# PRBonn/kinematic-icp

Measured on NVIDIA H100. Metric: scans/sec (full ICP), higher is better.
Workload: dtype f64

## Files before the change

kinematic-icp_b200/csrc/kicp_register.cu:

```cuda
#include <cfloat>
#include <cmath>
#include <cstddef>
#include <cstdio>
#include <cstdlib>
#include <cstring>
#include <algorithm>

#include "kicp_register.cuh"
#include "kicp_solve.cuh"

using namespace kicp_dev;

#ifndef KR_WARPS
#define KR_WARPS 10
#endif
#define KR_THREADS (KR_WARPS * 32)
#ifndef KR_MINB
#define KR_MINB 2
#endif
#ifndef KR_LCAP
#define KR_LCAP 192
#endif
#ifndef KR_G
#define KR_G 3
#endif
#ifndef KR_MERGE_MAX
#define KR_MERGE_MAX 19
#endif
#ifndef KR_SLOWWIN
#define KR_SLOWWIN 8
#endif
#define KR_CLASSES 4
#ifndef KR_CLS_HEAVY
#define KR_CLS_HEAVY 8
#endif
#ifndef KR_CLS_MID
#define KR_CLS_MID 4
#endif
#define KR_DBLMAX_BITS 0x7FEFFFFFFFFFFFFFull
#ifdef KR_PROFILE
#define KR_PROF_DECL long long prof_t[24] = {0}; long long prof_last = clock64(); int prof_o = 0;
#define KR_PROF(i) { const long long t__ = clock64(); prof_t[prof_o + (i)] += t__ - prof_last; prof_last = t__; }
#define KR_PROF_COUNT(i) { prof_t[prof_o + (i)] += 1; }
#define KR_PROF_PASS(it) { prof_o = (it) ? 12 : 0; }
#define KR_PROF_FLUSH if (lane == 0) { for (int k__ = 0; k__ < 24; ++k__) atomicAdd(&st->prof[k__], (unsigned long long)prof_t[k__]); }
#define KR_WLOG_CAP 65536
__device__ unsigned long long g_wlog[KR_WLOG_CAP][4];
__device__ unsigned int g_wlog_n;
__device__ __forceinline__ unsigned smid() { unsigned r; asm volatile("mov.u32 %0, %%smid;" : "=r"(r)); return r; }
#define KR_WLOG(kind, t0, t1, a_, b_) if (lane == 0) { const unsigned i__ = atomicAdd(&g_wlog_n, 1u); if (i__ < KR_WLOG_CAP) { \
    g_wlog[i__][0] = (t0), g_wlog[i__][1] = (t1); \
    g_wlog[i__][2] = ((unsigned long long)(kind) << 56) | ((unsigned long long)it << 48) | ((unsigned long long)smid() << 32) | gwarp; \
    g_wlog[i__][3] = ((unsigned long long)(unsigned)(a_) << 32) | (unsigned)(b_); } }
#define KR_WLOG_DO(x) x
#else
#define KR_WLOG(kind, t0, t1, a_, b_)
#define KR_WLOG_DO(x)
#define KR_PROF_DECL
#define KR_PROF(i)
#define KR_PROF_COUNT(i)
#define KR_PROF_PASS(it)
#define KR_PROF_FLUSH
#endif

struct RegState {
    PoseState pose;
    unsigned int win_ctr;
    unsigned int arrive;
    unsigned int exit_ctr;
    unsigned int ticket;
    unsigned int a_arrive;
    union {
        unsigned int cls_n[KR_CLASSES][KICP_MAX_ITERATIONS];
        struct { unsigned int slow_n[KICP_MAX_ITERATIONS], heavy_n[KICP_MAX_ITERATIONS], mid_n[KICP_MAX_ITERATIONS], todo_n[KICP_MAX_ITERATIONS]; };
    };
    int abort;
    int *iters_out;
    double acc[8];
    unsigned long long stats[4];
    unsigned long long prof[24];
    double dbg[KICP_MAX_ITERATIONS][6];
    kicp_reg_result result;
};

#ifndef KR_EMU
__device__ __forceinline__ unsigned long long gtime_ns() {
    unsigned long long t;
    asm volatile("mov.u64 %0, %%globaltimer;" : "=l"(t));
    return t;
}
__device__ __forceinline__ uint32_t ld_acquire_sys_u32(const uint32_t *p) {
    uint32_t v;
    asm volatile("ld.acquire.sys.global.u32 %0, [%1];" : "=r"(v) : "l"(p) : "memory");
    return v;
}
__device__ __forceinline__ unsigned int ld_acquire_gpu_u32(const unsigned int *p) {
    unsigned int v;
    asm volatile("ld.acquire.gpu.global.u32 %0, [%1];" : "=r"(v) : "l"(p) : "memory");
    return v;
}
__device__ __forceinline__ void st_relaxed_sys_u64(unsigned long long *p, unsigned long long v) {
    asm volatile("st.relaxed.sys.global.u64 [%0], %1;" ::"l"(p), "l"(v) : "memory");
}
__device__ __forceinline__ unsigned long long ld_relaxed_sys_u64(const unsigned long long *p) {
    unsigned long long v;
    asm volatile("ld.relaxed.sys.global.u64 %0, [%1];" : "=l"(v) : "l"(p) : "memory");
    return v;
}
#endif
struct __align__(32) Point4 {
    double x, y, z, w;
};
#ifndef KR_EMU
__device__ __forceinline__ Point4 ld_point(const double *p) {
    Point4 r;
    asm volatile("ld.global.nc.v2.f64 {%0, %1}, [%2];" : "=d"(r.x), "=d"(r.y) : "l"(p));
    asm volatile("ld.global.nc.f64 %0, [%1];" : "=d"(r.z) : "l"(p + 2));
    r.w = 0.0;
    return r;
}
#endif

__global__ void k_reg_init(RegState *st, RegArgs a) {
    if (threadIdx.x != 0 || blockIdx.x != 0) return;
    pose_init(&st->pose, a);
    result_init(&st->result, &st->pose);
    st->ticket = 0, st->win_ctr = 0, st->arrive = 0, st->exit_ctr = 0, st->abort = 0, st->a_arrive = 0;
    for (int c = 0; c < KR_CLASSES; ++c)
        for (int k = 0; k < KICP_MAX_ITERATIONS; ++k) st->cls_n[c][k] = 0;
    st->iters_out = a.iters_out;
    if (a.iters_out) *a.iters_out = 0;
    for (int k = 0; k < 8; ++k) st->acc[k] = 0.0;
}

__global__ void k_solve(RegState *st) {
    if (threadIdx.x == 0 && blockIdx.x == 0 && !st->pose.done) {
        double s[8];
        for (int k = 0; k < 8; ++k) s[k] = st->acc[k];
        solve_and_update(&st->pose, s, &st->result, st->iters_out);
        for (int k = 0; k < 8; ++k) st->acc[k] = 0.0;
    }
}

#define KR_TCAP 640
struct __align__(8) LineDesc {
    unsigned gline;
    unsigned short owner;
    unsigned short nvalid;
};
struct __align__(16) WarpSm {
    double2 qxy[32];
    double qz[32];
    double lmin[KR_LCAP];
    LineDesc ldesc[KR_LCAP];
    int vx[32], vy[32], vz[32];
    double acc[7][32];
    double px[32], py[32];
    unsigned short task[KR_TCAP];
};

__device__ __noinline__ bool same_norm(double a, double b) { return sqrt(a) == sqrt(b); }
__device__ __forceinline__ bool closer(double d2, double best) {
    if (!(d2 < best)) return false;
    if (d2 >= best * (1.0 - 4e-16)) return !same_norm(d2, best);
    return true;
}

__device__ __forceinline__ double dist2(double cx, double cy, double cz, double qx, double qy, double qz) {
    const double dx = cx - qx, dy = cy - qy, dz = cz - qz;
    return add_rn(add_rn(__dmul_rn(dx, dx), __dmul_rn(dy, dy)), __dmul_rn(dz, dz));
}

__device__ __forceinline__ void query_rn(const double q[4], const double t[3], double px, double py, double pz, double &ox, double &oy,
                                         double &oz) {
    quat_rotate_rn(q[0], q[1], q[2], q[3], px, py, pz, ox, oy, oz);
    ox = add_rn(ox, t[0]), oy = add_rn(oy, t[1]), oz = add_rn(oz, t[2]);
}

__device__ __forceinline__ void load_scan_point(const ScanView &sv, int i, double &x, double &y, double &z) {
    const unsigned char *p = sv.base + (size_t)i * (size_t)sv.stride;
    if (sv.f32) {
        x = (double)__ldg(reinterpret_cast<const float *>(p + sv.ox));
        y = (double)__ldg(reinterpret_cast<const float *>(p + sv.oy));
        z = (double)__ldg(reinterpret_cast<const float *>(p + sv.oz));
    } else {
        x = __ldg(reinterpret_cast<const double *>(p + sv.ox));
        y = __ldg(reinterpret_cast<const double *>(p + sv.oy));
        z = __ldg(reinterpret_cast<const double *>(p + sv.oz));
    }
}

__device__ __forceinline__ void stats_flush(RegState *st, unsigned long long probes, unsigned long long cands, unsigned long long lines) {
#pragma unroll
    for (int d = 16; d > 0; d >>= 1) {
        probes += __shfl_xor_sync(0xFFFFFFFFu, probes, d);
        cands += __shfl_xor_sync(0xFFFFFFFFu, cands, d);
        lines += __shfl_xor_sync(0xFFFFFFFFu, lines, d);
    }
    if ((threadIdx.x & 31) == 0) atomicAdd(&st->stats[0], probes), atomicAdd(&st->stats[1], cands), atomicAdd(&st->stats[2], lines);
}

__device__ __forceinline__ unsigned stage_mask(int stage, bool valid, double bound, double qx, double qy, double qz, int vx, int vy,
                                               int vz, double vs, double &minpruned) {
    if (!valid) return 0u;
    if (stage == 0) return 1u;
    double t;
    t = (double)(vx + 1) * vs - qx; const double gxp = t * t;
    t = qx - (double)vx * vs;       const double gxm = t * t;
    t = (double)(vy + 1) * vs - qy; const double gyp = t * t;
    t = qy - (double)vy * vs;       const double gym = t * t;
    t = (double)(vz + 1) * vs - qz; const double gzp = t * t;
    t = qz - (double)vz * vs;       const double gzm = t * t;
    if (stage == 1) {
        unsigned mask = 0u;
        if (gxp <= bound) mask |= 1u << 1; else minpruned = fmin(minpruned, gxp);
        if (gxm <= bound) mask |= 1u << 2; else minpruned = fmin(minpruned, gxm);
        if (gyp <= bound) mask |= 1u << 3; else minpruned = fmin(minpruned, gyp);
        if (gym <= bound) mask |= 1u << 4; else minpruned = fmin(minpruned, gym);
        if (gzp <= bound) mask |= 1u << 5; else minpruned = fmin(minpruned, gzp);
        if (gzm <= bound) mask |= 1u << 6; else minpruned = fmin(minpruned, gzm);
        return mask;
    }
    unsigned mask = 0u;
#pragma unroll
    for (int kk = 7; kk < 27; ++kk) {
        const double lb2 = (shift_x(kk) > 0 ? gxp : (shift_x(kk) < 0 ? gxm : 0.0)) + (shift_y(kk) > 0 ? gyp : (shift_y(kk) < 0 ? gym : 0.0)) +
                           (shift_z(kk) > 0 ? gzp : (shift_z(kk) < 0 ? gzm : 0.0));
        if (lb2 <= bound) mask |= 1u << kk; else minpruned = fmin(minpruned, lb2);
    }
    return mask;
}

__device__ __forceinline__ unsigned seeded_near_mask(double sd, double tau, double qx, double qy, double qz, int vx, int vy, int vz, double vs,
                                                     double &minpruned) {
    const double seed2 = sd * sd * (1.0 + 1e-6);
    const double bound = fmin(tau * tau, seed2) * (1.0 + 1e-6) + 1e-10;
    return stage_mask(1, true, bound, qx, qy, qz, vx, vy, vz, vs, minpruned) | stage_mask(2, true, bound, qx, qy, qz, vx, vy, vz, vs, minpruned);
}

__device__ __forceinline__ unsigned *class_entry(const KernelArgs &a, int n, int c, unsigned pos) {
    unsigned *const base = (c == 0 || c == 3) ? a.todo : a.todo2;
    return base + ((c & 1) ? pos : (unsigned)n - 1u - pos);
}

__device__ __forceinline__ void accumulate(WarpSm &sm, int lane, const PoseState &ps, double nx, double ny, double nz, double qx, double qy,
                                           double qz, double px, double py) {
    const double rx = qx - nx, ry = qy - ny, rz = qz - nz;
    const double rr = rx * rx + ry * ry + rz * rz;
    if (sqrt(rr) < ps.tau) {
        const double c0x = ps.R[0], c0y = ps.R[3], c0z = ps.R[6];
        const double c1x = ps.R[1] * px - ps.R[0] * py, c1y = ps.R[4] * px - ps.R[3] * py, c1z = ps.R[7] * px - ps.R[6] * py;
        sm.acc[0][lane] += c0x * c0x + c0y * c0y + c0z * c0z;
        sm.acc[1][lane] += c0x * c1x + c0y * c1y + c0z * c1z;
        sm.acc[2][lane] += c1x * c1x + c1y * c1y + c1z * c1z;
        sm.acc[3][lane] += c0x * rx + c0y * ry + c0z * rz;
        sm.acc[4][lane] += c1x * rx + c1y * ry + c1z * rz;
        sm.acc[5][lane] += 1.0;
        sm.acc[6][lane] += rr;
    }
}

__device__ __forceinline__ int voxel_of(double x, double vs, double inv_vs, int pow2) {
    return pow2 ? (int)floor(x * inv_vs) : voxel_coord(x, vs);
}

template <bool PERSISTENT>
__global__ void __launch_bounds__(KR_THREADS, KR_MINB) k_register(const KernelArgs a) {
#ifndef KR_EMU
    extern __shared__ __align__(16) unsigned char s_dyn[];
#else
    __shared__ __align__(16) unsigned char s_dyn[KR_WARPS * sizeof(WarpSm)];
#endif
    __shared__ PoseState s_ps;
    __shared__ double s_part[KR_WARPS][8];
    __shared__ double s_sum[8];
    __shared__ int s_flag[2];
    __shared__ volatile int s_ncls[2];

    const int lane = threadIdx.x & 31, wid = threadIdx.x >> 5;
    const int quad = lane >> 2, sub = lane & 3;
    const unsigned FULL = 0xFFFFFFFFu;
    WarpSm &sm = reinterpret_cast<WarpSm *>(s_dyn)[wid];
    RegState *const st = a.st;
    const int n = a.scan.d_n ? min(__ldg(a.scan.d_n), a.scan.n) : a.scan.n;
    const int num_windows = (n + 31) >> 5;
    const unsigned total_warps = gridDim.x * KR_WARPS;
    const unsigned gwarp = blockIdx.x * KR_WARPS + (threadIdx.x >> 5);

    if (threadIdx.x == 0) {
        if (PERSISTENT) {
            pose_init(&s_ps, a.init);
            if (blockIdx.x == 0) {
                result_init(&st->result, &s_ps);
                if (a.init.iters_out) *a.init.iters_out = 0;
            }
        } else {
            s_ps = st->pose;
        }
    }
    __syncthreads();
    if (!PERSISTENT && s_ps.done) return;

    unsigned long long n_probe = 0, n_cand = 0, n_line = 0;
    unsigned tbase = 0;
    KR_PROF_DECL

    for (unsigned it = 0; !s_ps.done; ++it) {
#pragma unroll
        for (int k = 0; k < 7; ++k) sm.acc[k][lane] = 0.0;
        const unsigned long long t_iter0 = gtime_ns();
        KR_PROF_PASS(it)
        const double inv_vs = 1.0 / a.map.voxel_size;
        const int tpb = max(1, min(32, KR_LCAP / ((a.map.cap + 3) >> 2)));
        const bool cache = PERSISTENT && a.nn_g != nullptr;
        unsigned tk = 0;
        int nsearch = num_windows;
        unsigned long long t_a1 = t_iter0, t_a2 = t_iter0;

        if (cache && it > 0u) {
            for (int w = (int)gwarp; w < num_windows; w += (int)total_warps) {
                const int i = w * 32 + lane;
                const bool valid = i < n;
                double px = 0, py = 0, pz = 0;
                if (valid) load_scan_point(a.scan, i, px, py, pz);
                const unsigned g1 = valid ? __ldcg(&a.nn_g[i]) : 0xFFFFFFFFu;
                const unsigned g2 = valid ? __ldcg(&a.nn_g2[i]) : 0xFFFFFFFFu;
                const double l = valid ? (double)__ldcg(&a.nn_l[i]) : 0.0;
                const bool haveg = g1 != 0xFFFFFFFFu, have2 = g2 != 0xFFFFFFFFu;
                const Point4 c1 = ld_point(a.map.pts + (size_t)(haveg ? g1 : 0u) * KICP_PSTRIDE);
                const Point4 c2 = ld_point(a.map.pts + (size_t)(have2 ? g2 : 0u) * KICP_PSTRIDE);
                double qx, qy, qz, ox, oy, oz;
                query_rn(s_ps.q, s_ps.t, px, py, pz, qx, qy, qz);
                query_rn(s_ps.qp, s_ps.tp, px, py, pz, ox, oy, oz);
                const double vs = a.map.voxel_size;
                const int vx = voxel_of(qx, vs, inv_vs, a.pow2_voxel), vy = voxel_of(qy, vs, inv_vs, a.pow2_voxel),
                          vz = voxel_of(qz, vs, inv_vs, a.pow2_voxel);
                const int ovx = voxel_of(ox, vs, inv_vs, a.pow2_voxel), ovy = voxel_of(oy, vs, inv_vs, a.pow2_voxel),
                          ovz = voxel_of(oz, vs, inv_vs, a.pow2_voxel);
                const double mx = qx - ox, my = qy - oy, mz = qz - oz;
                const double delta = sqrt(mx * mx + my * my + mz * mz) * (1.0 + 1e-9) + 1e-12;
                const double d1 = sqrt(dist2(c1.x, c1.y, c1.z, qx, qy, qz));
                const double d2 = have2 ? sqrt(dist2(c2.x, c2.y, c2.z, qx, qy, qz)) : DBL_MAX;
                const bool second_wins = d2 < d1;
                const double dn = second_wins ? d2 : d1;
                const bool clear = !have2 || fabs(d1 - d2) > 1e-9 * (d1 + d2) + 1e-12;
                const Point4 c = second_wins ? c2 : c1;
                double slab = DBL_MAX;
                bool reach = true;
                if (vx != ovx || vy != ovy || vz != ovz) {
                    reach = abs(vx - ovx) <= 1 && abs(vy - ovy) <= 1 && abs(vz - ovz) <= 1;
                    if (vx > ovx) slab = fmin(slab, (double)(vx + 1) * vs - qx); else if (vx < ovx) slab = fmin(slab, qx - (double)vx * vs);
                    if (vy > ovy) slab = fmin(slab, (double)(vy + 1) * vs - qy); else if (vy < ovy) slab = fmin(slab, qy - (double)vy * vs);
                    if (vz > ovz) slab = fmin(slab, (double)(vz + 1) * vs - qz); else if (vz < ovz) slab = fmin(slab, qz - (double)vz * vs);
                    if (haveg)
                        reach = reach && abs(voxel_of(c1.x, vs, inv_vs, a.pow2_voxel) - vx) <= 1 && abs(voxel_of(c1.y, vs, inv_vs, a.pow2_voxel) - vy) <= 1 &&
                                abs(voxel_of(c1.z, vs, inv_vs, a.pow2_voxel) - vz) <= 1;
                    if (have2)
                        reach = reach && abs(voxel_of(c2.x, vs, inv_vs, a.pow2_voxel) - vx) <= 1 && abs(voxel_of(c2.y, vs, inv_vs, a.pow2_voxel) - vy) <= 1 &&
                                abs(voxel_of(c2.z, vs, inv_vs, a.pow2_voxel) - vz) <= 1;
                }
                const double room = fmin(l - delta, slab * (1.0 - 1e-9) - 1e-12);
                const bool cert = valid && reach && (haveg ? (clear && dn * (1.0 + 1e-9) + 1e-12 < room) : (room > s_ps.tau * (1.0 + 1e-9)));
                if (cert) {
                    a.nn_l[i] = __double2float_rz(room * (1.0 - 1e-7));
                    if (second_wins) a.nn_g[i] = g2, a.nn_g2[i] = g1;
                    if (haveg) accumulate(sm, lane, s_ps, c.x, c.y, c.z, qx, qy, qz, px, py);
                }
                const bool again = valid && !cert;
                int cls = -1;
                if (again) {
                    float seed = 3.0e38f;
                    if (haveg && abs(voxel_of(c.x, vs, inv_vs, a.pow2_voxel) - vx) <= 1 && abs(voxel_of(c.y, vs, inv_vs, a.pow2_voxel) - vy) <= 1 &&
                        abs(voxel_of(c.z, vs, inv_vs, a.pow2_voxel) - vz) <= 1)
                        seed = __double2float_ru(dn * (1.0 + 1e-7));
                    a.nn_l[i] = seed;
                    cls = 0;
                    if (seed < 1.0e38f) {
                        double mp = DBL_MAX;
                        const int near = __popc(seeded_near_mask((double)seed, s_ps.tau, qx, qy, qz, vx, vy, vz, vs, mp));
                        if (near <= KR_MERGE_MAX) cls = near + 1 >= KR_CLS_HEAVY ? 1 : near + 1 >= KR_CLS_MID ? 2 : 3;
                    }
                }
                unsigned need = 0u, cnt = 0u;
#pragma unroll
                for (int k = 0; k < KR_CLASSES; ++k) {
                    const unsigned m = __ballot_sync(FULL, cls == k);
                    if (cls == k) need = m;
                    if (lane == k) cnt = m;
                }
                unsigned pos = 0;
                if (cnt) pos = atomicAdd(&st->cls_n[lane][it], (unsigned)__popc(cnt));
                pos = __shfl_sync(FULL, pos, max(cls, 0)) + (unsigned)__popc(need & ((1u << lane) - 1u));
                if (cls >= 0) *class_entry(a, n, cls, pos) = (unsigned)i;
            }
            KR_WLOG(1, t_iter0, gtime_ns(), 0, 0)
            __syncthreads();
            if (threadIdx.x == 0) {
                t_a1 = gtime_ns();
                __threadfence();
                atomicAdd(&st->a_arrive, 1u);
                const unsigned target = it * gridDim.x;
                const unsigned long long deadline = gtime_ns() + a.timeout_ns;
                while (ld_acquire_gpu_u32(&st->a_arrive) < target) {
                    __nanosleep(20);
                    if (gtime_ns() > deadline) {
                        atomicExch(&st->abort, KICP_ERR_CUDA);
                        break;
                    }
                }
                t_a2 = gtime_ns();
                s_ncls[0] = (int)__ldcg(&st->cls_n[1][it]), s_ncls[1] = (int)__ldcg(&st->cls_n[2][it]);
            }
            __syncthreads();
        }
        const bool indirect = cache && it > 0u;
        const int nfast = indirect ? (int)(__ldcg(&st->cls_n[1][it]) + __ldcg(&st->cls_n[2][it]) + __ldcg(&st->cls_n[3][it])) : n;
        const int nslow = indirect ? (int)__ldcg(&st->cls_n[0][it]) : 0;
        const int P = (int)total_warps;
        const int nslowwin = (nslow + KR_SLOWWIN - 1) / KR_SLOWWIN;
        const int Pf = max(P - nslowwin, P / 2);
        int wsz = 32;
        if (PERSISTENT && nfast > 0) {
            if (nfast <= 32 * Pf) {
                wsz = max(1, (nfast + Pf - 1) / Pf);
            } else {
                const int rounds = (nfast + 32 * (P + nslowwin) - 1) / (32 * P);
                wsz = min(32, (nfast + rounds * Pf - 1) / (rounds * Pf));
            }
        }
        const int segpts = max(32, ((((n + 31) >> 5) + KICP_UPLOAD_CHUNKS - 1) / KICP_UPLOAD_CHUNKS) * 32);
        const int segwin = (segpts + wsz - 1) / wsz;
        int nfastwin;
        if (indirect) {
            nfastwin = (nfast + wsz - 1) / wsz;
        } else {
            const int nseg = min(KICP_UPLOAD_CHUNKS, (n + segpts - 1) / segpts), lastn = n - (nseg - 1) * segpts;
            nfastwin = n > 0 ? (nseg - 1) * segwin + (lastn + wsz - 1) / wsz : 0;
        }
        nsearch = nslowwin + nfastwin;

        int w = min((int)gwarp, nsearch);
        const unsigned dyn = (unsigned)max(nsearch - (int)total_warps, 0);
        KR_PROF(11)
        while (w < nsearch) {
            if (lane == 0) tk = atomicAdd(&st->win_ctr, 1u);
            KR_PROF_COUNT(8)
            KR_WLOG_DO(const unsigned long long wl_t0 = gtime_ns(); unsigned wl_tasks = 0; unsigned wl_lines = 0;)
            int slot, limit, seg_of_w = 0, wlanes = wsz, cls = 0;
            if (indirect) {
                if (w < nslowwin) {
                    slot = lane * nslowwin + w, limit = nslow, wlanes = KR_SLOWWIN;
                } else {
                    slot = lane * nfastwin + (w - nslowwin), limit = nfast, cls = 1;
                }
            } else {
                const int sgi = min(w / segwin, KICP_UPLOAD_CHUNKS - 1), lw = w - sgi * segwin;
                const int sbase = sgi * segpts, sn = min(segpts, n - sbase);
                const int sw = (sn + wsz - 1) / wsz;
                slot = sbase + lane * sw + lw, limit = lw < sw ? sbase + sn : 0;
                seg_of_w = sgi;
            }
            const bool valid = lane < wlanes && slot < limit;
            int pi = valid ? slot : 0;
            if (indirect) {
                int pos = slot;
                if (cls == 1 && pos >= s_ncls[0]) pos -= s_ncls[0], cls = 2;
                if (cls == 2 && pos >= s_ncls[1]) pos -= s_ncls[1], cls = 3;
                pi = valid ? (int)__ldcg(class_entry(a, n, cls, (unsigned)pos)) : 0;
            }
            if (PERSISTENT && a.up.flags != nullptr && it == 0u) {
                const uint32_t *f = a.up.flags + seg_of_w;
                const unsigned long long deadline = gtime_ns() + a.timeout_ns;
                bool pend = true;
                while (__any_sync(FULL, pend)) {
                    if (pend) {
                        if (ld_acquire_sys_u32(f) == a.up.seq) {
                            pend = false;
                        } else if (gtime_ns() > deadline) {
                            if (lane == 0) atomicExch(&st->abort, KICP_ERR_CUDA);
                            pend = false;
                        }
                    }
                }
            }
            double seed2 = DBL_MAX, seed_d = 3.0e38;
            {
                double px = 0, py = 0, pz = 0;
                if (valid) load_scan_point(a.scan, pi, px, py, pz);
                if (indirect && valid) {
                    const double sd = (double)__ldcg(&a.nn_l[pi]);
                    if (sd < 1.0e38) seed_d = sd, seed2 = sd * sd * (1.0 + 1e-6);
                }
                double qx, qy, qz;
                query_rn(s_ps.q, s_ps.t, px, py, pz, qx, qy, qz);
                sm.qxy[lane] = make_double2(qx, qy), sm.qz[lane] = qz;
                sm.vx[lane] = voxel_of(qx, a.map.voxel_size, inv_vs, a.pow2_voxel);
                sm.vy[lane] = voxel_of(qy, a.map.voxel_size, inv_vs, a.pow2_voxel);
                sm.vz[lane] = voxel_of(qz, a.map.voxel_size, inv_vs, a.pow2_voxel);
                sm.px[lane] = px, sm.py[lane] = py;
            }
            double best = DBL_MAX, second = DBL_MAX, third = DBL_MAX, minpruned = DBL_MAX;
            unsigned bline = 0xFFFFFFFFu, bvalid = 0u;
            unsigned sline = 0xFFFFFFFFu, svalid = 0u;
            __syncwarp();
            KR_PROF(0)

            unsigned donem = 0u;
            bool merged = false;
            for (int stage = 0; stage < 3; ++stage) {
                if (stage == 1 && !__any_sync(FULL, valid && !merged)) break;
                int total, tfirst, tcount;
                {
                    const double2 qq = sm.qxy[lane];
                    const double tau2 = s_ps.tau * s_ps.tau;
                    const double bsq = fmin(fmin(tau2, best), seed2);
                    const double bound = bsq * (1.0 + 1e-6) + 1e-10;
                    unsigned mask = stage_mask(stage, valid, bound, qq.x, qq.y, sm.qz[lane], sm.vx[lane], sm.vy[lane], sm.vz[lane],
                                               a.map.voxel_size, minpruned);
                    if (stage == 0 && valid && seed_d < 1.0e38) {
                        double mp = minpruned;
                        const unsigned near = seeded_near_mask(seed_d, s_ps.tau, qq.x, qq.y, sm.qz[lane], sm.vx[lane], sm.vy[lane], sm.vz[lane],
                                                               a.map.voxel_size, mp);
                        if (__popc(near) <= KR_MERGE_MAX) mask |= near, minpruned = mp, merged = true;
                    }
                    mask &= ~donem;
                    donem |= mask;
                    const int no = __popc(mask);
                    int tin = no;
#pragma unroll
                    for (int d = 1; d < 32; d <<= 1) {
                        const int y = __shfl_up_sync(FULL, tin, d);
                        if (lane >= d) tin += y;
                    }
                    total = __shfl_sync(FULL, tin, 31);
                    int pos = tin - no;
                    tfirst = pos, tcount = no;
                    const int maxno = __reduce_max_sync(FULL, no);
                    for (int i = 0; i < maxno; ++i) {
                        if (mask) {
                            const int k = __ffs(mask) - 1;
                            mask &= mask - 1;
                            sm.task[pos++] = (unsigned short)((lane << 5) | k);
                        }
                    }
                    __syncwarp();
                }
                KR_PROF(1)
                KR_WLOG_DO(wl_tasks += (unsigned)total;)
                int fill = 0, lbase = 0;
                int olb = 0, ole = 0;
                bool ohas = false;
                for (int base = 0;; base += tpb) {
                    const bool more = base < total;
                    const bool act = more && lane < tpb && base + lane < total;
                    const unsigned okpack = act ? (unsigned)sm.task[base + lane] : 0u;
                    uint32_t meta = KICP_SLOT_EMPTY;
                    if (more) {
                        KR_PROF_COUNT(9)
                        const int o = (int)(okpack >> 5), k = (int)(okpack & 31u);
                        const int kx = sm.vx[o] + shift_x(k), ky = sm.vy[o] + shift_y(k), kz = sm.vz[o] + shift_z(k);
                        uint32_t h = voxel_hash(kx, ky, kz) & a.map.mask;
                        const int4 s0 = __ldg(&a.map.slots[h]);
                        const int4 s1 = __ldg(&a.map.slots[(h + 1) & a.map.mask]);
                        bool pend = false;
                        if (act && (uint32_t)s0.w != KICP_SLOT_EMPTY) {
                            if (s0.x == kx && s0.y == ky && s0.z == kz) {
                                meta = (uint32_t)s0.w;
                            } else if ((uint32_t)s1.w != KICP_SLOT_EMPTY) {
                                if (s1.x == kx && s1.y == ky && s1.z == kz) {
                                    meta = (uint32_t)s1.w;
                                } else {
                                    pend = true, h = (h + 2) & a.map.mask;
                                }
                            }
                        }
                        while (__any_sync(FULL, pend)) {
                            if (pend) {
                                const int4 sl = __ldg(&a.map.slots[h]);
                                if ((uint32_t)sl.w == KICP_SLOT_EMPTY) {
                                    pend = false;
                                } else if (sl.x == kx && sl.y == ky && sl.z == kz) {
                                    meta = (uint32_t)sl.w, pend = false;
                                } else {
                                    h = (h + 1) & a.map.mask;
                                }
                            }
                        }
                    }
                    KR_PROF(2)
                    const int cnt = meta == KICP_SLOT_EMPTY ? 0 : (int)(meta & 0xFFu);
                    const int nl = (cnt + 3) >> 2;
                    int incl = nl;
#pragma unroll
                    for (int d = 1; d < 32; d <<= 1) {
                        const int y = __shfl_up_sync(FULL, incl, d);
                        if (lane >= d) incl += y;
                    }
                    const int ltot = __shfl_sync(FULL, incl, 31);
                    if (a.collect_stats) n_probe += act ? 1 : 0, n_cand += cnt, n_line += nl;

                    if ((!more || fill + ltot > KR_LCAP) && fill > 0) {
                        KR_PROF(3)
                        for (int r0 = 0; r0 < fill; r0 += 8 * KR_G) {
                            unsigned own[KR_G], gix[KR_G];
                            unsigned hasm = 0;
#pragma unroll
                            for (int g = 0; g < KR_G; ++g) {
                                const int line = r0 + g * 8 + quad;
                                LineDesc ld;
                                ld.gline = 0u, ld.owner = 0, ld.nvalid = 0;
                                if (line < fill) ld = sm.ldesc[line];
                                const bool has = sub < (int)ld.nvalid;
                                own[g] = ld.owner;
                                gix[g] = ld.gline + (has ? (unsigned)sub : 0u);
                                hasm |= has ? (1u << g) : 0u;
                            }
                            Point4 c[KR_G];
#pragma unroll
                            for (int g = 0; g < KR_G; ++g) c[g] = ld_point(a.map.pts + (size_t)gix[g] * KICP_PSTRIDE);
                            KR_PROF_COUNT(10)
                            KR_PROF(4)
#pragma unroll
                            for (int g = 0; g < KR_G; ++g) {
                                const double2 qq = sm.qxy[own[g]];
                                double d2 = (hasm >> g) & 1u ? dist2(c[g].x, c[g].y, c[g].z, qq.x, qq.y, sm.qz[own[g]]) : DBL_MAX;
                                d2 = fmin(d2, __shfl_xor_sync(FULL, d2, 1));
                                d2 = fmin(d2, __shfl_xor_sync(FULL, d2, 2));
                                if (sub == 0 && r0 + g * 8 + quad < fill) sm.lmin[r0 + g * 8 + quad] = d2;
                            }
                        }
                        __syncwarp();
                        {
                            const int lb = ohas ? max(olb - lbase, 0) : 0, le = ohas ? min(ole - lbase, fill) : 0;
                            const int maxlen = __reduce_max_sync(FULL, max(le - lb, 0));
                            for (int u = 0; u < maxlen; ++u) {
                                if (lb + u < le) {
                                    const double dl = sm.lmin[lb + u];
                                    if (closer(dl, best)) {
                                        const LineDesc ld = sm.ldesc[lb + u];
                                        third = second;
                                        second = best, sline = bline, svalid = bvalid;
                                        best = dl, bline = ld.gline, bvalid = ld.nvalid;
                                    } else if (dl < second) {
                                        const LineDesc ld = sm.ldesc[lb + u];
                                        third = second;
                                        second = dl, sline = ld.gline, svalid = ld.nvalid;
                                    } else {
                                        third = fmin(third, dl);
                                    }
                                }
                            }
                        }
                        __syncwarp();
                        KR_WLOG_DO(wl_lines += (unsigned)fill;)
                        lbase += fill, fill = 0;
                        KR_PROF(5)
                    }
                    if (!more) break;
                    {
                        const int gl = lbase + fill + (incl - nl);
                        const int t0 = max(tfirst - base, 0), t1 = min(tfirst + tcount - base, tpb);
                        const int b0 = __shfl_sync(FULL, gl, t0 & 31), e1 = __shfl_sync(FULL, gl + nl, (t1 - 1) & 31);
                        if (t1 > t0) {
                            if (!ohas) olb = b0, ohas = true;
                            ole = e1;
                        }
                        const int maxnl = __reduce_max_sync(FULL, nl);
                        for (int li = 0; li < maxnl; ++li) {
                            if (li < nl) {
                                LineDesc ld;
                                ld.gline = (meta >> 8) * (unsigned)a.map.cap + (unsigned)(li * 4);
                                ld.owner = (unsigned short)(okpack >> 5);
                                ld.nvalid = (unsigned short)min(cnt - li * 4, 4);
                                sm.ldesc[gl - lbase + li] = ld;
                            }
                        }
                        fill += ltot;
                    }
                    __syncwarp();
                    KR_PROF(3)
                }
                __syncwarp();
            }
            KR_PROF(1)
            {
                const bool have = valid && bline != 0xFFFFFFFFu;
                const unsigned g0 = have ? bline : 0u;
                Point4 cc[4];
#pragma unroll
                for (int j = 0; j < 4; ++j) cc[j] = ld_point(a.map.pts + (size_t)(g0 + (j < (int)bvalid ? j : 0)) * KICP_PSTRIDE);
                const double2 q0 = sm.qxy[lane];
                const double q0z = sm.qz[lane];
                double dj[4];
#pragma unroll
                for (int j = 0; j < 4; ++j) dj[j] = dist2(cc[j].x, cc[j].y, cc[j].z, q0.x, q0.y, q0z);
                int jw = 0;
#pragma unroll
                for (int j = 1; j < 4; ++j)
                    if (j < (int)bvalid && closer(dj[j], dj[jw])) jw = j;
                Point4 c = cc[0];
#pragma unroll
                for (int j = 1; j < 4; ++j)
                    if (jw == j) c = cc[j];
                if (have) accumulate(sm, lane, s_ps, c.x, c.y, c.z, q0.x, q0.y, q0z, sm.px[lane], sm.py[lane]);
                if (cache && valid) {
                    const bool have2 = have && sline != 0xFFFFFFFFu;
                    Point4 ce[4];
#pragma unroll
                    for (int j = 0; j < 4; ++j) ce[j] = ld_point(a.map.pts + (size_t)((have2 ? sline : 0u) + (j < (int)svalid ? j : 0)) * KICP_PSTRIDE);
                    double ru = DBL_MAX, ru2 = DBL_MAX;
                    unsigned g2 = 0xFFFFFFFFu;
#pragma unroll
                    for (int j = 0; j < 4; ++j) {
                        if (have && j < (int)bvalid && j != jw) {
                            if (dj[j] < ru) ru2 = ru, ru = dj[j], g2 = g0 + (unsigned)j;
                            else ru2 = fmin(ru2, dj[j]);
                        }
                    }
#pragma unroll
                    for (int j = 0; j < 4; ++j) {
                        const double de = dist2(ce[j].x, ce[j].y, ce[j].z, q0.x, q0.y, q0z);
                        if (have2 && j < (int)svalid) {
                            if (de < ru) ru2 = ru, ru = de, g2 = sline + (unsigned)j;
                            else ru2 = fmin(ru2, de);
                        }
                    }
                    const double lo2 = fmin(fmin(ru2, third), minpruned);
                    a.nn_g[pi] = have ? g0 + (unsigned)jw : 0xFFFFFFFFu;
                    a.nn_g2[pi] = g2;
                    a.nn_l[pi] = lo2 >= 1.0e60 ? 1.0e30f : __double2float_rz(sqrt(lo2) * (1.0 - 1e-7));
                }
            }
            __syncwarp();
            KR_PROF(6)
            KR_WLOG_DO(const unsigned wl_pts = (unsigned)__popc(__ballot_sync(FULL, valid));)
            KR_WLOG(0, wl_t0, gtime_ns(), (wl_tasks << 8) | wl_pts, wl_lines)
            w = (int)(total_warps + min(__shfl_sync(FULL, tk, 0) - tbase, dyn));
            KR_PROF(7)
        }
        tbase += (unsigned)nsearch;
        KR_PROF(11)

        const unsigned long long t_win = gtime_ns();
        double v[7];
#pragma unroll
        for (int k = 0; k < 7; ++k) v[k] = sm.acc[k][lane];
#pragma unroll
        for (int k = 0; k < 7; ++k) {
#pragma unroll
            for (int d = 16; d > 0; d >>= 1) v[k] += __shfl_xor_sync(FULL, v[k], d);
        }
        if (lane == 0) {
#pragma unroll
            for (int k = 0; k < 7; ++k) s_part[wid][k] = v[k];
            s_part[wid][7] = 0.0;
        }
        __syncthreads();
        double *const part = a.partials + (size_t)(PERSISTENT ? (it & 1u) : 0u) * gridDim.x * 8;
        if (threadIdx.x < 8) {
            double s = 0.0;
            for (int k = 0; k < KR_WARPS; ++k) s += s_part[k][threadIdx.x];
            __stcg(&part[(size_t)blockIdx.x * 8 + threadIdx.x], s);
            __threadfence();
        }
        __syncthreads();

        if (!PERSISTENT) {
            if (threadIdx.x == 0) {
                const unsigned ticket = atomicAdd(&st->ticket, 1u);
                s_flag[0] = (ticket == gridDim.x - 1);
            }
            __syncthreads();
            if (s_flag[0]) {
                __threadfence();
                if (threadIdx.x < 8) {
                    double s = 0.0;
                    for (unsigned bb = 0; bb < gridDim.x; ++bb) s += __ldcg(&part[(size_t)bb * 8 + threadIdx.x]);
                    st->acc[threadIdx.x] = s;
                }
                if (threadIdx.x == 0) st->ticket = 0, st->win_ctr = 0;
            }
            if (a.collect_stats) stats_flush(st, n_probe, n_cand, n_line);
            return;
        }

        const bool multi = a.px.nranks > 1;
        unsigned long long t_arr = 0, t_red = 0;
        if (threadIdx.x == 0) {
            atomicAdd(&st->arrive, 1u);
            if (!multi || blockIdx.x == 0) {
                const unsigned target = (it + 1u) * gridDim.x;
                const unsigned long long deadline = t_win + a.timeout_ns;
                while (ld_acquire_gpu_u32(&st->arrive) < target) {
                    __nanosleep(40);
                    if (gtime_ns() > deadline) {
                        atomicExch(&st->abort, KICP_ERR_CUDA);
                        break;
                    }
                }
            }
            t_arr = gtime_ns();
        }
        __syncthreads();
        if (!multi || blockIdx.x == 0) {
            const int col = threadIdx.x & 7, row0 = threadIdx.x >> 3;
            double s = 0.0;
            const unsigned nrow = (gridDim.x + KR_THREADS / 8 - 1) / (KR_THREADS / 8);
            for (unsigned kr = 0; kr < nrow; ++kr) {
                const unsigned bb = kr * (KR_THREADS / 8) + (unsigned)row0;
                if (bb < gridDim.x) s += __ldcg(&part[(size_t)bb * 8 + col]);
            }
            s += __shfl_xor_sync(FULL, s, 8);
            s += __shfl_xor_sync(FULL, s, 16);
            if (lane < 8) s_part[wid][lane] = s;
            __syncthreads();
            if (threadIdx.x < 8) {
                double tsum = 0.0;
                for (int k = 0; k < KR_WARPS; ++k) tsum += s_part[k][threadIdx.x];
                s_sum[threadIdx.x] = tsum;
            }
            __syncthreads();
        }
        if (multi) {
            const uint32_t tag = a.px.tag_base + it;
            if (wid == 0) {
                if (blockIdx.x == 0) {
                    const double val = s_sum[(lane & 15) >> 1];
                    const unsigned long long bits = (unsigned long long)__double_as_longlong(val);
                    const uint32_t half = (lane & 1) ? (uint32_t)(bits >> 32) : (uint32_t)bits;
                    const unsigned long long word = ((unsigned long long)tag << 32) | half;
#pragma unroll 1
                    for (int r = 0; r < a.px.nranks; ++r) {
                        st_relaxed_sys_u64(&a.px.peer[r]->ll[a.px.parity][it][a.px.rank][lane & 15], word);
                        __syncwarp();
                    }
                }
                __syncwarp();
                double tot = 0.0;
                bool timed_out = false;
                const unsigned long long deadline = gtime_ns() + a.timeout_ns;
                for (int r = 0; r < a.px.nranks; ++r) {
                    unsigned long long wv = 0;
                    const unsigned long long *src = &a.px.peer[a.px.rank]->ll[a.px.parity][it][r][lane & 15];
                    bool pend = true;
                    while (__any_sync(FULL, pend)) {
                        if (pend) {
                            wv = ld_relaxed_sys_u64(src);
                            if ((uint32_t)(wv >> 32) == tag) {
                                pend = false;
                            } else if (gtime_ns() > deadline) {
                                timed_out = true, pend = false;
                            }
                        }
                    }
                    const uint32_t lo = __shfl_sync(FULL, (uint32_t)wv, (lane & 7) * 2);
                    const uint32_t hi = __shfl_sync(FULL, (uint32_t)wv, (lane & 7) * 2 + 1);
                    tot += __longlong_as_double((long long)(((unsigned long long)hi << 32) | lo));
                }
                timed_out = __any_sync(FULL, timed_out);
                if (lane < 8) s_sum[lane] = tot;
                if (lane == 0) s_flag[1] = timed_out ? 1 : 0;
            }
            __syncthreads();
        }
        if (threadIdx.x == 0) {
            t_red = gtime_ns();
            int ab = (int)ld_acquire_gpu_u32((const unsigned int *)&st->abort);
            if (!ab && multi && s_flag[1]) ab = KICP_ERR_NCCL;
            if (ab) {
                s_ps.status = ab, s_ps.done = 1;
                if (blockIdx.x == 0) st->result.status = ab;
            } else {
                double s[8];
                for (int k = 0; k < 8; ++k) s[k] = s_sum[k];
                solve_and_update(&s_ps, s, blockIdx.x == 0 ? &st->result : nullptr, blockIdx.x == 0 ? a.init.iters_out : nullptr);
            }
            if (blockIdx.x == 0 && it < KICP_MAX_ITERATIONS) {
                st->dbg[it][0] = (double)(t_a1 - t_iter0), st->dbg[it][1] = (double)(t_a2 - t_a1), st->dbg[it][2] = (double)(t_win - t_a2);
                st->dbg[it][3] = (double)(t_arr - t_win), st->dbg[it][4] = (double)(t_red - t_arr), st->dbg[it][5] = (double)(gtime_ns() - t_red);
            }
        }
        __syncthreads();
    }

    if (PERSISTENT) {
        if (a.collect_stats) stats_flush(st, n_probe, n_cand, n_line);
        KR_PROF_FLUSH
        __syncthreads();
        if (blockIdx.x == 0 && a.result_host != nullptr) {
            const double *src = reinterpret_cast<const double *>(&st->result);
            double *dst = reinterpret_cast<double *>(a.result_host);
            for (unsigned i = threadIdx.x; i < sizeof(kicp_reg_result) / sizeof(double); i += KR_THREADS) dst[i] = __ldcg(src + i);
            __threadfence_system();
        }
        if (threadIdx.x == 0) {
            __threadfence();
            const unsigned left = atomicAdd(&st->exit_ctr, 1u);
            if (left == gridDim.x - 1) {
                st->win_ctr = 0, st->arrive = 0, st->abort = 0, st->a_arrive = 0;
                for (int c = 0; c < KR_CLASSES; ++c)
                    for (int k = 0; k < KICP_MAX_ITERATIONS; ++k) st->cls_n[c][k] = 0;
                __threadfence();
                st->exit_ctr = 0;
            }
        }
    }
}


#ifndef KR_EMU
__global__ void k_l2_read(const uint4 *__restrict__ p, size_t n, int reps, unsigned *sink) {
    unsigned acc = 0;
    for (int r = 0; r < reps; ++r)
        for (size_t i = (size_t)blockIdx.x * blockDim.x + threadIdx.x; i < n; i += (size_t)gridDim.x * blockDim.x) {
            const uint4 v = __ldcg(p + i);
            acc += v.x ^ v.y ^ v.z ^ v.w;
        }
    if (acc == 0x12345678u) *sink = acc;
}
size_t kr_state_bytes() { return sizeof(RegState); }
size_t kr_offset_result() { return offsetof(RegState, result); }
size_t kr_offset_acc() { return offsetof(RegState, acc); }
size_t kr_offset_dbg() { return offsetof(RegState, dbg); }
size_t kr_offset_stats() { return offsetof(RegState, stats); }
size_t kr_stats_bytes() { return sizeof(((RegState *)0)->stats) + sizeof(((RegState *)0)->prof); }
size_t kr_smem_bytes() { return (size_t)KR_WARPS * sizeof(WarpSm); }

cudaError_t kr_prepare(int *persistent_ctas_per_sm, int *multilaunch_ctas_per_sm) {
    cudaError_t e = cudaFuncSetAttribute(k_register<true>, cudaFuncAttributeMaxDynamicSharedMemorySize, (int)kr_smem_bytes());
    if (e == cudaSuccess) e = cudaFuncSetAttribute(k_register<false>, cudaFuncAttributeMaxDynamicSharedMemorySize, (int)kr_smem_bytes());
    if (e == cudaSuccess) e = cudaOccupancyMaxActiveBlocksPerMultiprocessor(persistent_ctas_per_sm, k_register<true>, KR_THREADS, kr_smem_bytes());
    if (e == cudaSuccess) e = cudaOccupancyMaxActiveBlocksPerMultiprocessor(multilaunch_ctas_per_sm, k_register<false>, KR_THREADS, kr_smem_bytes());
    return e;
}
cudaError_t kr_launch_init(RegState *st, const RegArgs &a, cudaStream_t stream) {
    k_reg_init<<<1, 32, 0, stream>>>(st, a);
    return cudaGetLastError();
}
cudaError_t kr_launch_solve(RegState *st, cudaStream_t stream) {
    k_solve<<<1, 32, 0, stream>>>(st);
    return cudaGetLastError();
}
cudaError_t kr_window_log(unsigned long long *out, size_t cap_entries, size_t *n) {
    *n = 0;
#ifdef KR_PROFILE
    unsigned cnt = 0;
    cudaError_t e = cudaMemcpyFromSymbol(&cnt, g_wlog_n, sizeof(cnt));
    if (e != cudaSuccess) return e;
    *n = std::min<size_t>(std::min<size_t>(cnt, KR_WLOG_CAP), cap_entries);
    return cudaMemcpyFromSymbol(out, g_wlog, *n * 4 * sizeof(unsigned long long));
#else
    (void)out, (void)cap_entries;
    return cudaSuccess;
#endif
}
cudaError_t kr_launch_register(bool persistent, int grid, KernelArgs &ka, cudaStream_t stream) {
#ifdef KR_PROFILE
    {
        void *p = nullptr;
        cudaGetSymbolAddress(&p, g_wlog_n);
        cudaMemsetAsync(p, 0, sizeof(unsigned), stream);
    }
#endif
    if (persistent) {
        void *args[] = {&ka};
        return cudaLaunchCooperativeKernel((const void *)k_register<true>, dim3(grid), dim3(KR_THREADS), args, kr_smem_bytes(), stream);
    }
    k_register<false><<<grid, KR_THREADS, kr_smem_bytes(), stream>>>(ka);
    return cudaGetLastError();
}
cudaError_t kr_launch_l2_read(const void *buf, size_t bytes, int reps, unsigned *sink, int grid, cudaStream_t stream) {
    k_l2_read<<<grid, 256, 0, stream>>>((const uint4 *)buf, bytes / 16, reps, sink);
    return cudaGetLastError();
}
#endif
```

Measured before the change: 3027.

## Batch cached-certify windows per warp with prefetch and one atomic per sweep

The cached-correspondence certify pass now handles up to eight grid-strided windows per warp in a sweep. It prefetches the next window's scan point and cached indices while certifying the current one. Class counts are accumulated across the sweep, so one atomicAdd per class reserves slots for all windows, followed by a second pass that writes the class entries. The abort flag is also read right after the arrival spin rather than with a separate acquire load later, which could weaken memory ordering for the single-rank path.

```diff
diff --git a/kinematic-icp_b200/csrc/kicp_register.cu b/kinematic-icp_b200/csrc/kicp_register.cu
--- a/kinematic-icp_b200/csrc/kicp_register.cu
+++ b/kinematic-icp_b200/csrc/kicp_register.cu
@@ -31,6 +31,7 @@
 #define KR_SLOWWIN 8
 #endif
 #define KR_CLASSES 4
+#define KR_SWEEP 8
 #ifndef KR_CLS_HEAVY
 #define KR_CLS_HEAVY 8
 #endif
@@ -264,6 +265,64 @@
     return pow2 ? (int)floor(x * inv_vs) : voxel_coord(x, vs);
 }
 
+__device__ __forceinline__ int certify(const KernelArgs &a, const PoseState &ps, WarpSm &sm, int lane, int i, bool valid, double px, double py,
+                                       double pz, unsigned g1, unsigned g2, double l, const Point4 &c1, const Point4 &c2, double inv_vs) {
+    const bool haveg = g1 != 0xFFFFFFFFu, have2 = g2 != 0xFFFFFFFFu;
+    double qx, qy, qz, ox, oy, oz;
+    query_rn(ps.q, ps.t, px, py, pz, qx, qy, qz);
+    query_rn(ps.qp, ps.tp, px, py, pz, ox, oy, oz);
+    const double vs = a.map.voxel_size;
+    const int vx = voxel_of(qx, vs, inv_vs, a.pow2_voxel), vy = voxel_of(qy, vs, inv_vs, a.pow2_voxel),
+              vz = voxel_of(qz, vs, inv_vs, a.pow2_voxel);
+    const int ovx = voxel_of(ox, vs, inv_vs, a.pow2_voxel), ovy = voxel_of(oy, vs, inv_vs, a.pow2_voxel),
+              ovz = voxel_of(oz, vs, inv_vs, a.pow2_voxel);
+    const double mx = qx - ox, my = qy - oy, mz = qz - oz;
+    const double delta = sqrt(mx * mx + my * my + mz * mz) * (1.0 + 1e-9) + 1e-12;
+    const double d1 = sqrt(dist2(c1.x, c1.y, c1.z, qx, qy, qz));
+    const double d2 = have2 ? sqrt(dist2(c2.x, c2.y, c2.z, qx, qy, qz)) : DBL_MAX;
+    const bool second_wins = d2 < d1;
+    const double dn = second_wins ? d2 : d1;
+    const bool clear = !have2 || fabs(d1 - d2) > 1e-9 * (d1 + d2) + 1e-12;
+    const Point4 c = second_wins ? c2 : c1;
+    double slab = DBL_MAX;
+    bool reach = true;
+    if (vx != ovx || vy != ovy || vz != ovz) {
+        reach = abs(vx - ovx) <= 1 && abs(vy - ovy) <= 1 && abs(vz - ovz) <= 1;
+        if (vx > ovx) slab = fmin(slab, (double)(vx + 1) * vs - qx); else if (vx < ovx) slab = fmin(slab, qx - (double)vx * vs);
+        if (vy > ovy) slab = fmin(slab, (double)(vy + 1) * vs - qy); else if (vy < ovy) slab = fmin(slab, qy - (double)vy * vs);
+        if (vz > ovz) slab = fmin(slab, (double)(vz + 1) * vs - qz); else if (vz < ovz) slab = fmin(slab, qz - (double)vz * vs);
+        if (haveg)
+            reach = reach && abs(voxel_of(c1.x, vs, inv_vs, a.pow2_voxel) - vx) <= 1 && abs(voxel_of(c1.y, vs, inv_vs, a.pow2_voxel) - vy) <= 1 &&
+                    abs(voxel_of(c1.z, vs, inv_vs, a.pow2_voxel) - vz) <= 1;
+        if (have2)
+            reach = reach && abs(voxel_of(c2.x, vs, inv_vs, a.pow2_voxel) - vx) <= 1 && abs(voxel_of(c2.y, vs, inv_vs, a.pow2_voxel) - vy) <= 1 &&
+                    abs(voxel_of(c2.z, vs, inv_vs, a.pow2_voxel) - vz) <= 1;
+    }
+    const double room = fmin(l - delta, slab * (1.0 - 1e-9) - 1e-12);
+    const bool cert = valid && reach && (haveg ? (clear && dn * (1.0 + 1e-9) + 1e-12 < room) : (room > ps.tau * (1.0 + 1e-9)));
+    if (cert) {
+        a.nn_l[i] = __double2float_rz(room * (1.0 - 1e-7));
+        if (second_wins) a.nn_g[i] = g2, a.nn_g2[i] = g1;
+        if (haveg) accumulate(sm, lane, ps, c.x, c.y, c.z, qx, qy, qz, px, py);
+    }
+    const bool again = valid && !cert;
+    int cls = -1;
+    if (again) {
+        float seed = 3.0e38f;
+        if (haveg && abs(voxel_of(c.x, vs, inv_vs, a.pow2_voxel) - vx) <= 1 && abs(voxel_of(c.y, vs, inv_vs, a.pow2_voxel) - vy) <= 1 &&
+            abs(voxel_of(c.z, vs, inv_vs, a.pow2_voxel) - vz) <= 1)
+            seed = __double2float_ru(dn * (1.0 + 1e-7));
+        a.nn_l[i] = seed;
+        cls = 0;
+        if (seed < 1.0e38f) {
+            double mp = DBL_MAX;
+            const int near = __popc(seeded_near_mask((double)seed, ps.tau, qx, qy, qz, vx, vy, vz, vs, mp));
+            if (near <= KR_MERGE_MAX) cls = near + 1 >= KR_CLS_HEAVY ? 1 : near + 1 >= KR_CLS_MID ? 2 : 3;
+        }
+    }
+    return cls;
+}
+
 template <bool PERSISTENT>
 __global__ void __launch_bounds__(KR_THREADS, KR_MINB) k_register(const KernelArgs a) {
 #ifndef KR_EMU
@@ -318,80 +377,49 @@
         unsigned long long t_a1 = t_iter0, t_a2 = t_iter0;
 
         if (cache && it > 0u) {
-            for (int w = (int)gwarp; w < num_windows; w += (int)total_warps) {
-                const int i = w * 32 + lane;
-                const bool valid = i < n;
+            for (int w0 = (int)gwarp; w0 < num_windows; w0 += KR_SWEEP * (int)total_warps) {
+                const int kn = min(KR_SWEEP, (num_windows - 1 - w0) / (int)total_warps + 1);
+                int i = w0 * 32 + lane;
                 double px = 0, py = 0, pz = 0;
-                if (valid) load_scan_point(a.scan, i, px, py, pz);
-                const unsigned g1 = valid ? __ldcg(&a.nn_g[i]) : 0xFFFFFFFFu;
-                const unsigned g2 = valid ? __ldcg(&a.nn_g2[i]) : 0xFFFFFFFFu;
-                const double l = valid ? (double)__ldcg(&a.nn_l[i]) : 0.0;
-                const bool haveg = g1 != 0xFFFFFFFFu, have2 = g2 != 0xFFFFFFFFu;
-                const Point4 c1 = ld_point(a.map.pts + (size_t)(haveg ? g1 : 0u) * KICP_PSTRIDE);
-                const Point4 c2 = ld_point(a.map.pts + (size_t)(have2 ? g2 : 0u) * KICP_PSTRIDE);
-                double qx, qy, qz, ox, oy, oz;
-                query_rn(s_ps.q, s_ps.t, px, py, pz, qx, qy, qz);
-                query_rn(s_ps.qp, s_ps.tp, px, py, pz, ox, oy, oz);
-                const double vs = a.map.voxel_size;
-                const int vx = voxel_of(qx, vs, inv_vs, a.pow2_voxel), vy = voxel_of(qy, vs, inv_vs, a.pow2_voxel),
-                          vz = voxel_of(qz, vs, inv_vs, a.pow2_voxel);
-                const int ovx = voxel_of(ox, vs, inv_vs, a.pow2_voxel), ovy = voxel_of(oy, vs, inv_vs, a.pow2_voxel),
-                          ovz = voxel_of(oz, vs, inv_vs, a.pow2_voxel);
-                const double mx = qx - ox, my = qy - oy, mz = qz - oz;
-                const double delta = sqrt(mx * mx + my * my + mz * mz) * (1.0 + 1e-9) + 1e-12;
-                const double d1 = sqrt(dist2(c1.x, c1.y, c1.z, qx, qy, qz));
-                const double d2 = have2 ? sqrt(dist2(c2.x, c2.y, c2.z, qx, qy, qz)) : DBL_MAX;
-                const bool second_wins = d2 < d1;
-                const double dn = second_wins ? d2 : d1;
-                const bool clear = !have2 || fabs(d1 - d2) > 1e-9 * (d1 + d2) + 1e-12;
-                const Point4 c = second_wins ? c2 : c1;
-                double slab = DBL_MAX;
-                bool reach = true;
-                if (vx != ovx || vy != ovy || vz != ovz) {
-                    reach = abs(vx - ovx) <= 1 && abs(vy - ovy) <= 1 && abs(vz - ovz) <= 1;
-                    if (vx > ovx) slab = fmin(slab, (double)(vx + 1) * vs - qx); else if (vx < ovx) slab = fmin(slab, qx - (double)vx * vs);
-                    if (vy > ovy) slab = fmin(slab, (double)(vy + 1) * vs - qy); else if (vy < ovy) slab = fmin(slab, qy - (double)vy * vs);
-                    if (vz > ovz) slab = fmin(slab, (double)(vz + 1) * vs - qz); else if (vz < ovz) slab = fmin(slab, qz - (double)vz * vs);
-                    if (haveg)
-                        reach = reach && abs(voxel_of(c1.x, vs, inv_vs, a.pow2_voxel) - vx) <= 1 && abs(voxel_of(c1.y, vs, inv_vs, a.pow2_voxel) - vy) <= 1 &&
-                                abs(voxel_of(c1.z, vs, inv_vs, a.pow2_voxel) - vz) <= 1;
-                    if (have2)
-                        reach = reach && abs(voxel_of(c2.x, vs, inv_vs, a.pow2_voxel) - vx) <= 1 && abs(voxel_of(c2.y, vs, inv_vs, a.pow2_voxel) - vy) <= 1 &&
-                                abs(voxel_of(c2.z, vs, inv_vs, a.pow2_voxel) - vz) <= 1;
-                }
-                const double room = fmin(l - delta, slab * (1.0 - 1e-9) - 1e-12);
-                const bool cert = valid && reach && (haveg ? (clear && dn * (1.0 + 1e-9) + 1e-12 < room) : (room > s_ps.tau * (1.0 + 1e-9)));
-                if (cert) {
-                    a.nn_l[i] = __double2float_rz(room * (1.0 - 1e-7));
-                    if (second_wins) a.nn_g[i] = g2, a.nn_g2[i] = g1;
-                    if (haveg) accumulate(sm, lane, s_ps, c.x, c.y, c.z, qx, qy, qz, px, py);
-                }
-                const bool again = valid && !cert;
-                int cls = -1;
-                if (again) {
-                    float seed = 3.0e38f;
-                    if (haveg && abs(voxel_of(c.x, vs, inv_vs, a.pow2_voxel) - vx) <= 1 && abs(voxel_of(c.y, vs, inv_vs, a.pow2_voxel) - vy) <= 1 &&
-                        abs(voxel_of(c.z, vs, inv_vs, a.pow2_voxel) - vz) <= 1)
-                        seed = __double2float_ru(dn * (1.0 + 1e-7));
-                    a.nn_l[i] = seed;
-                    cls = 0;
-                    if (seed < 1.0e38f) {
-                        double mp = DBL_MAX;
-                        const int near = __popc(seeded_near_mask((double)seed, s_ps.tau, qx, qy, qz, vx, vy, vz, vs, mp));
-                        if (near <= KR_MERGE_MAX) cls = near + 1 >= KR_CLS_HEAVY ? 1 : near + 1 >= KR_CLS_MID ? 2 : 3;
-                    }
-                }
-                unsigned need = 0u, cnt = 0u;
-#pragma unroll
-                for (int k = 0; k < KR_CLASSES; ++k) {
-                    const unsigned m = __ballot_sync(FULL, cls == k);
-                    if (cls == k) need = m;
-                    if (lane == k) cnt = m;
-                }
-                unsigned pos = 0;
-                if (cnt) pos = atomicAdd(&st->cls_n[lane][it], (unsigned)__popc(cnt));
-                pos = __shfl_sync(FULL, pos, max(cls, 0)) + (unsigned)__popc(need & ((1u << lane) - 1u));
-                if (cls >= 0) *class_entry(a, n, cls, pos) = (unsigned)i;
+                if (i < n) load_scan_point(a.scan, i, px, py, pz);
+                unsigned g1 = i < n ? __ldcg(&a.nn_g[i]) : 0xFFFFFFFFu, g2 = i < n ? __ldcg(&a.nn_g2[i]) : 0xFFFFFFFFu;
+                float l = i < n ? __ldcg(&a.nn_l[i]) : 0.0f;
+                unsigned clsp = 0u;
+                unsigned ccnt = 0u;
+#pragma unroll 1
+                for (int k = 0; k < kn; ++k) {
+                    const Point4 c1 = ld_point(a.map.pts + (size_t)(g1 != 0xFFFFFFFFu ? g1 : 0u) * KICP_PSTRIDE);
+                    const Point4 c2 = ld_point(a.map.pts + (size_t)(g2 != 0xFFFFFFFFu ? g2 : 0u) * KICP_PSTRIDE);
+                    const int inext = k + 1 < kn ? i + (int)total_warps * 32 : n;
+                    double nx = 0, ny = 0, nz = 0;
+                    if (inext < n) load_scan_point(a.scan, inext, nx, ny, nz);
+                    const unsigned n1 = inext < n ? __ldcg(&a.nn_g[inext]) : 0xFFFFFFFFu, n2 = inext < n ? __ldcg(&a.nn_g2[inext]) : 0xFFFFFFFFu;
+                    const float nl = inext < n ? __ldcg(&a.nn_l[inext]) : 0.0f;
+                    const int cls = certify(a, s_ps, sm, lane, i, i < n, px, py, pz, g1, g2, (double)l, c1, c2, inv_vs);
+                    clsp |= (unsigned)(cls + 1) << (4 * k);
+#pragma unroll
+                    for (int c = 0; c < KR_CLASSES; ++c) {
+                        const unsigned m = __ballot_sync(FULL, cls == c);
+                        if (lane == c) ccnt += (unsigned)__popc(m);
+                    }
+                    i += (int)total_warps * 32, px = nx, py = ny, pz = nz, g1 = n1, g2 = n2, l = nl;
+                }
+                unsigned next = 0u;
+                if (ccnt) next = atomicAdd(&st->cls_n[lane][it], ccnt);
+#pragma unroll 1
+                for (int k = 0; k < kn; ++k) {
+                    const int cls = (int)((clsp >> (4 * k)) & 15u) - 1;
+                    unsigned need = 0u, cnt = 0u;
+#pragma unroll
+                    for (int c = 0; c < KR_CLASSES; ++c) {
+                        const unsigned m = __ballot_sync(FULL, cls == c);
+                        if (cls == c) need = m;
+                        if (lane == c) cnt = m;
+                    }
+                    const unsigned pos = __shfl_sync(FULL, next, max(cls, 0)) + (unsigned)__popc(need & ((1u << lane) - 1u));
+                    next += (unsigned)__popc(cnt);
+                    if (cls >= 0) *class_entry(a, n, cls, pos) = (unsigned)((w0 + k * (int)total_warps) * 32 + lane);
+                }
             }
             KR_WLOG(1, t_iter0, gtime_ns(), 0, 0)
             __syncthreads();
@@ -786,6 +814,7 @@
 
         const bool multi = a.px.nranks > 1;
         unsigned long long t_arr = 0, t_red = 0;
+        int ab = 0;
         if (threadIdx.x == 0) {
             atomicAdd(&st->arrive, 1u);
             if (!multi || blockIdx.x == 0) {
@@ -798,6 +827,7 @@
                         break;
                     }
                 }
+                ab = __ldcg(&st->abort);
             }
             t_arr = gtime_ns();
         }
@@ -865,7 +895,7 @@
         }
         if (threadIdx.x == 0) {
             t_red = gtime_ns();
-            int ab = (int)ld_acquire_gpu_u32((const unsigned int *)&st->abort);
+            if (multi && blockIdx.x != 0) ab = (int)ld_acquire_gpu_u32((const unsigned int *)&st->abort);
             if (!ab && multi && s_flag[1]) ab = KICP_ERR_NCCL;
             if (ab) {
                 s_ps.status = ab, s_ps.done = 1;
```

Result: no change. 3057 (median of 6 runs) (+1.0%).
